# Agzs/BlockMaze

Hardware: AMD Instinct MI355X
Metric: Groth16 proofs/sec (send circuit, alt_bn128) (higher is better)
Workload: dtype u32 limbs (254-bit Fq/Fr Montgomery; all MSM accumulations, the H query's weighted bucket sum and the transforms' tiles on nine 29-bit limbs)

## Files before the change

### blockmaze_amd/csrc/msm.cuh

```cuda
#pragma once
#include <hip/hip_runtime.h>
#include "curve.cuh"

#include "field29.cuh"
namespace zk { struct MsmCounters { uint32_t n_ones; uint32_t n_other; uint32_t pad[2]; }; }
#include "htail29.cuh"
#include "oct29.cuh"
namespace zk {

constexpr int MSM_MAX_WINDOWS = 64;

__host__ __device__ inline int msm_num_windows(int c) { return 254 / c + 1; }

__device__ __forceinline__ void signed_digits(const uint32_t k[8], int c, int W, int *dig) {
  uint32_t carry = 0; const uint32_t half = 1u << (c - 1), full = 1u << c, mask = full - 1;
  for (int w = 0; w < W; w++) {
    int bit = w * c, word = bit >> 5, sh = bit & 31;
    uint64_t v = word < 8 ? k[word] : 0; if (word + 1 < 8) v |= (uint64_t)k[word + 1] << 32;
    uint32_t d = ((uint32_t)(v >> sh) & mask) + carry;
    if (d > half) { dig[w] = (int)d - (int)full; carry = 1; } else { dig[w] = (int)d; carry = 0; }
  }
}

template <int C, class Fn> __device__ __forceinline__ void for_each_digit(const uint32_t (&k)[8], Fn &&fn) {
// ... 12 lines not shown
}
constexpr uint32_t MSM_ENTRY_SIGN = 0x80000000u;


constexpr uint32_t MSM_LDS_HIST = 4096;
template <int C>
__global__ void __launch_bounds__(256) k_msm_classify(const Fr *__restrict__ scalars, const uint32_t *__restrict__ scalar_index,
    const uint8_t *__restrict__ point_is_inf,
                               uint32_t n, int c, int W, int filter_ones, uint32_t hist_stride, uint32_t n_hist, uint32_t *__restrict__ hist,
                                   uint32_t *__restrict__ ones, MsmCounters *cnt, MsmCounters *cnt_next) {
  __shared__ uint32_t lh[MSM_LDS_HIST]; const bool use_lds = n_hist <= MSM_LDS_HIST;
  if (blockIdx.x == 0 && threadIdx.x == 0) *cnt_next = MsmCounters{0, 0, {0, 0}};
  if (use_lds) { for (uint32_t b = threadIdx.x; b < n_hist; b += blockDim.x) lh[b] = 0; __syncthreads(); }
  uint32_t i = blockIdx.x * blockDim.x + threadIdx.x; bool live = i < n && !(point_is_inf && point_is_inf[i]); Fr k = Fr::zero();
  if (live) { k = scalars[scalar_index ? scalar_index[i] : i].from_mont(); live = !k.is_zero(); }
  bool is_one = false; if (live && filter_ones) { uint32_t o = k.l[0] ^ 1u; for (int j = 1; j < 8; j++) o |= k.l[j]; is_one = o == 0; }
  {
    uint64_t m = __ballot(is_one);
    if (m) {
      uint32_t lane = threadIdx.x & 63, base = 0;
      if (lane == (uint32_t)__ffsll((long long)m) - 1) base = atomicAdd(&cnt->n_ones, (uint32_t)__popcll(m));
      base = __shfl(base, __ffsll((long long)m) - 1, 64); if (is_one) ones[base + __popcll(m & ((1ull << lane) - 1))] = i; } }
  if (live && !is_one)
    msm_walk_digits<C>(k.l, c, W, [&](int w, int d) { if (d) { uint32_t key = (uint32_t)w * hist_stride + (uint32_t)(d < 0 ? -d : d) - 1;
        atomicAdd(use_lds ? &lh[key] : &hist[key], 1u); } });
  {
    uint64_t m = __ballot(live && !is_one);
    if (m && (threadIdx.x & 63) == (uint32_t)__ffsll((long long)m) - 1) atomicAdd(&cnt->n_other, (uint32_t)__popcll(m));
  }
  if (use_lds) { __syncthreads(); for (uint32_t b = threadIdx.x; b < n_hist; b += blockDim.x) if (lh[b]) atomicAdd(&hist[b], lh[b]); }
}

template <int C>
__global__ void __launch_bounds__(256) k_msm_scatter(const Fr *__restrict__ scalars, const uint32_t *__restrict__ scalar_index,
    const uint8_t *__restrict__ point_is_inf,
                              uint32_t n, int c, int W, int filter_ones, uint32_t hist_stride, uint32_t point_stride, uint32_t n_hist,
                                  const uint32_t *__restrict__ offsets, uint32_t *__restrict__ fill, uint32_t *__restrict__ entries) {
  __shared__ uint32_t lcnt[MSM_LDS_HIST], lbase[MSM_LDS_HIST]; const bool use_lds = n_hist <= MSM_LDS_HIST;
  if (use_lds) { for (uint32_t b = threadIdx.x; b < n_hist; b += blockDim.x) lcnt[b] = 0; __syncthreads(); }
  uint32_t i = blockIdx.x * blockDim.x + threadIdx.x; bool live = i < n && !(point_is_inf && point_is_inf[i]); Fr k = Fr::zero();
  if (live) { k = scalars[scalar_index ? scalar_index[i] : i].from_mont(); live = !k.is_zero(); }
  if (live && filter_ones) { uint32_t o = k.l[0] ^ 1u; for (int j = 1; j < 8; j++) o |= k.l[j]; if (o == 0) live = false; }
  auto entry_of = [&](int w, int d) {
    return (i + (uint32_t)w * point_stride) | (d < 0 ? MSM_ENTRY_SIGN : 0u);
  };
  if (!use_lds) {
    if (live) msm_walk_digits<C>(k.l, c, W, [&](int w, int d) { if (!d) return; uint32_t key = (uint32_t)w * hist_stride + (uint32_t)(d < 0 ? -d : d) - 1;
        entries[offsets[key] + atomicAdd(&fill[key], 1u)] = entry_of(w, d); });
    return;
  }
  if (live) msm_walk_digits<C>(k.l, c, W, [&](int w, int d) { if (d) atomicAdd(&lcnt[(uint32_t)w * hist_stride + (uint32_t)(d < 0 ? -d : d) - 1], 1u); });
  __syncthreads();
  for (uint32_t b = threadIdx.x; b < n_hist; b += blockDim.x) {
    const uint32_t m = lcnt[b];
    lbase[b] = m ? offsets[b] + atomicAdd(&fill[b], m) : 0;
    lcnt[b] = 0;
  }
  __syncthreads();
  if (live) msm_walk_digits<C>(k.l, c, W, [&](int w, int d) { if (!d) return; uint32_t key = (uint32_t)w * hist_stride + (uint32_t)(d < 0 ? -d : d) - 1;
      entries[lbase[key] + atomicAdd(&lcnt[key], 1u)] = entry_of(w, d); });
}

__host__ __device__ inline uint32_t hsort_spread(int c) { const int W = 254 / c + 1, tb = 254 - c * (W - 1); return tb < c - 2 && c * W > 256 ? 1u << (c * W - 256) : 1u; }
__host__ __device__ inline uint32_t hsort_multiple(uint32_t i, uint32_t spread) { return spread > 1 ? ((i * 2654435761u) >> 16) % spread : 0u; }
__device__ __forceinline__ void signed_digits9(const uint32_t k[9], int c, int W, int *dig) {
  uint32_t carry = 0; const uint32_t half = 1u << (c - 1), full = 1u << c, mask = full - 1;
  for (int w = 0; w < W; w++) {
    int bit = w * c, word = bit >> 5, sh = bit & 31;
    uint64_t v = word < 9 ? k[word] : 0; if (word + 1 < 9) v |= (uint64_t)k[word + 1] << 32;
    uint32_t d = ((uint32_t)(v >> sh) & mask) + carry;
    if (d > half) { dig[w] = (int)d - (int)full; carry = 1; } else { dig[w] = (int)d; carry = 0; }
  }
}
template <int C, class Fn> __device__ __forceinline__ void hsort_walk_digits(const uint32_t (&k)[8], uint32_t i, uint32_t spread, int c, int W, Fn &&fn) {
  if constexpr (C > 0) { msm_walk_digits<C>(k, c, W, fn); }
  else {
    const uint32_t m = hsort_multiple(i, spread); uint32_t k9[9]; uint64_t carry = 0;
#pragma unroll
    for (int j = 0; j < 8; j++) { const uint64_t t = (uint64_t)k[j] + (uint64_t)m * FrParams::MOD[j] + carry; k9[j] = (uint32_t)t; carry = t >> 32; }
    k9[8] = (uint32_t)carry;
    int dig[MSM_MAX_WINDOWS]; signed_digits9(k9, c, W, dig); for (int w = 0; w < W; w++) fn(w, dig[w]);
  }
}
constexpr uint32_t HSORT_GROUPS = 1024 , HSORT_BIN_THREADS = 256, HSORT_PER_THREAD = 2,
    HSORT_TILE = HSORT_BIN_THREADS * HSORT_PER_THREAD, HSORT_GROUP_THREADS = 1024, HSORT_MAX_PER_THREAD = 24, HSORT_SLICES = 8,
    HSORT_STAGE_W = 20 ;
struct HsortShape { uint32_t groups, low_bits, idx_bits, region; };
template <int C>
__global__ void __launch_bounds__(HSORT_BIN_THREADS) k_hsort_bin(const Fr *__restrict__ scalars, const Fr *__restrict__ mul_b, const Fr *__restrict__ mul_z,
    int z_is_table, const uint8_t *__restrict__ point_is_inf,
                                                                 uint32_t n, int c, int W, uint32_t point_stride, HsortShape sh, uint32_t spread,
                                                                     uint32_t *__restrict__ group_fill, uint32_t *__restrict__ mid, MsmCounters *cnt,
                                                                     MsmCounters *cnt_next) {
  zk_take_prio(sh.low_bits);
  __shared__ uint32_t lcnt[HSORT_GROUPS], lpos[HSORT_GROUPS], gbase[HSORT_GROUPS];
  __shared__ uint32_t stage[HSORT_TILE * HSORT_STAGE_W];
  __shared__ uint16_t stage_g[HSORT_TILE * HSORT_STAGE_W];
  __shared__ uint32_t wave_tot[HSORT_BIN_THREADS / 64];
  if (blockIdx.x == 0 && threadIdx.x == 0) *cnt_next = MsmCounters{0, 0, {0, 0}};
  for (uint32_t g = threadIdx.x; g < sh.groups; g += blockDim.x) lcnt[g] = 0;
  __syncthreads();
  Fr k[HSORT_PER_THREAD]; bool live[HSORT_PER_THREAD];
#pragma unroll
  for (int q = 0; q < (int)HSORT_PER_THREAD; q++) {
    const uint32_t i = blockIdx.x * HSORT_TILE + q * HSORT_BIN_THREADS + threadIdx.x;
    live[q] = i < n && !(point_is_inf && point_is_inf[i]);
    k[q] = Fr::zero();
    if (live[q]) { Fr v = scalars[i]; if (mul_b) v = v * mul_b[i] * mul_z[z_is_table ? i : 0]; k[q] = v.from_mont(); live[q] = !k[q].is_zero(); } }
  const uint32_t low_mask = (1u << sh.low_bits) - 1;
#pragma unroll
  for (int q = 0; q < (int)HSORT_PER_THREAD; q++) if (live[q]) hsort_walk_digits<C>(k[q].l, blockIdx.x * HSORT_TILE + q * HSORT_BIN_THREADS + threadIdx.x, spread, c, W, [&](int, int d) {
      if (d) atomicAdd(&lcnt[((uint32_t)(d < 0 ? -d : d) - 1) >> sh.low_bits], 1u); });
  __syncthreads();
  {
    uint32_t s = 0;
    const uint32_t per = (sh.groups + HSORT_BIN_THREADS - 1) / HSORT_BIN_THREADS, lo = threadIdx.x * per;
    for (uint32_t j = 0; j < per; j++) if (lo + j < sh.groups) s += lcnt[lo + j];
    uint32_t inc = s; for (int d = 1; d < 64; d <<= 1) { uint32_t t = __shfl_up(inc, d, 64); if ((int)(threadIdx.x & 63) >= d) inc += t; }
    if ((threadIdx.x & 63) == 63) wave_tot[threadIdx.x >> 6] = inc;
    __syncthreads();
    uint32_t ex = inc - s; for (uint32_t wv = 0; wv < (threadIdx.x >> 6); wv++) ex += wave_tot[wv];
    bool over = false;
    for (uint32_t j = 0; j < per; j++) if (lo + j < sh.groups) {
      const uint32_t g = lo + j, m = lcnt[g];
      lpos[g] = ex;
      ex += m;
      const uint32_t b = m ? atomicAdd(&group_fill[g], m) : 0;
      if (b + m > sh.region) over = true;
      gbase[g] = b;
    }
    if (over) atomicOr(&cnt->pad[0], 1u); }
  __syncthreads();
  for (uint32_t g = threadIdx.x; g < sh.groups; g += blockDim.x) lcnt[g] = lpos[g];
  __syncthreads();
#pragma unroll
  for (int q = 0; q < (int)HSORT_PER_THREAD; q++) if (live[q]) { const uint32_t i = blockIdx.x * HSORT_TILE + q * HSORT_BIN_THREADS + threadIdx.x;
    hsort_walk_digits<C>(k[q].l, i, spread, c, W, [&](int w, int d) { if (!d) return; const uint32_t key = (uint32_t)(d < 0 ? -d : d) - 1, g = key >> sh.low_bits,
        p = atomicAdd(&lcnt[g], 1u);
      if (p < HSORT_TILE * HSORT_STAGE_W) { stage[p] = ((key & low_mask) << (sh.idx_bits + 1)) | ((d < 0 ? 1u : 0u) << sh.idx_bits) | (i +
          (uint32_t)w * point_stride); stage_g[p] = (uint16_t)g; } }); }
  __syncthreads();
  const uint32_t total = min(lcnt[sh.groups - 1], HSORT_TILE * HSORT_STAGE_W);
  for (uint32_t p = threadIdx.x; p < total; p += blockDim.x) {
    const uint32_t g = stage_g[p], pos = gbase[g] + (p - lpos[g]);
    if (pos < sh.region) mid[(size_t)g * sh.region + pos] = stage[p];
  }
}
static __global__ void __launch_bounds__(HSORT_GROUP_THREADS) k_hsort_group(const uint32_t *__restrict__ mid, uint32_t *__restrict__ group_fill, HsortShape sh,
    uint32_t *__restrict__ entries, uint32_t *__restrict__ counts, uint32_t *__restrict__ offsets,
                                                                            uint32_t *__restrict__ group_n) {
  zk_take_prio(sh.low_bits);
  __shared__ uint32_t lcnt[1024], lpre[1024];
  const uint32_t g = blockIdx.x, nb = 1u << sh.low_bits, n_g = min(group_fill[g], sh.region); const uint32_t *src = mid + (size_t)g * sh.region;
  for (uint32_t b = threadIdx.x; b < nb; b += blockDim.x) lcnt[b] = 0;
  __syncthreads();
  if (threadIdx.x == 0) {
    group_fill[g] = 0;
    group_n[g] = n_g;
  }
  uint32_t e[HSORT_MAX_PER_THREAD]; int ne = 0;
#pragma unroll
  for (int j = 0; j < (int)HSORT_MAX_PER_THREAD; j++) {
    const uint32_t p = (uint32_t)j * HSORT_GROUP_THREADS + threadIdx.x;
    if (p < n_g) {
      e[j] = src[p];
      atomicAdd(&lcnt[e[j] >> (sh.idx_bits + 1)], 1u);
      ne = j + 1;
    }
  }
  __syncthreads();
  if (threadIdx.x < 64) {
    const uint32_t per = (nb + 63) / 64, lo = threadIdx.x * per; uint32_t s = 0; for (uint32_t j = 0; j < per; j++) if (lo + j < nb) s += lcnt[lo + j];
    uint32_t inc = s; for (int d = 1; d < 64; d <<= 1) { uint32_t t = __shfl_up(inc, d, 64); if ((int)threadIdx.x >= d) inc += t; }
    uint32_t ex = inc - s; for (uint32_t j = 0; j < per; j++) if (lo + j < nb) { lpre[lo + j] = ex; ex += lcnt[lo + j]; } }
  __syncthreads();
  for (uint32_t b = threadIdx.x; b < nb; b += blockDim.x) {
    const uint32_t bucket = (g << sh.low_bits) | b;
    counts[bucket] = lcnt[b];
    offsets[bucket] = g * sh.region + lpre[b];
    lcnt[b] = 0;
  }
  __syncthreads();
  uint32_t *dst = entries + (size_t)g * sh.region;
  extern __shared__ uint32_t hsg_stage[];
#pragma unroll
  for (int j = 0; j < (int)HSORT_MAX_PER_THREAD; j++) if (j < ne) {
    const uint32_t v = e[j], b = v >> (sh.idx_bits + 1), r = atomicAdd(&lcnt[b], 1u);
    hsg_stage[lpre[b] + r] = v;
  }
  __syncthreads();
  for (uint32_t p = threadIdx.x; p < n_g; p += blockDim.x) dst[p] = hsg_stage[p];
}

static __global__ void k_fr_mul3(const Fr *__restrict__ a, const Fr *__restrict__ b, const Fr *__restrict__ z, int z_is_table, uint32_t n,
    Fr *__restrict__ out) {
  uint32_t i = blockIdx.x * blockDim.x + threadIdx.x; if (i < n) out[i] = a[i] * b[i] * z[z_is_table ? i : 0];
}

constexpr int SCAN_BLOCK = 1024, SCAN_ITEMS = 4;
static __global__ void k_scan_local(const uint32_t *__restrict__ in, uint32_t *__restrict__ out, uint32_t *__restrict__ block_sums, uint32_t n) {
  __shared__ uint32_t sh[SCAN_BLOCK]; uint32_t base = blockIdx.x * SCAN_BLOCK * SCAN_ITEMS + threadIdx.x * SCAN_ITEMS; uint32_t v[SCAN_ITEMS], s = 0;
  for (int j = 0; j < SCAN_ITEMS; j++) { v[j] = base + j < n ? in[base + j] : 0; s += v[j]; }
  sh[threadIdx.x] = s; __syncthreads();
  for (int d = 1; d < SCAN_BLOCK; d <<= 1) { uint32_t t = threadIdx.x >= d ? sh[threadIdx.x - d] : 0; __syncthreads(); sh[threadIdx.x] += t; __syncthreads(); }
  uint32_t excl = sh[threadIdx.x] - s;
  for (int j = 0; j < SCAN_ITEMS; j++) { if (base + j < n) out[base + j] = excl; excl += v[j]; }
  if (threadIdx.x == SCAN_BLOCK - 1) block_sums[blockIdx.x] = sh[SCAN_BLOCK - 1];
}
static __global__ void k_scan_block_sums(uint32_t *block_sums, uint32_t nblocks) {
  __shared__ uint32_t sh[SCAN_BLOCK]; uint32_t carry = 0;
  for (uint32_t base = 0; base < nblocks; base += SCAN_BLOCK) {
    uint32_t i = base + threadIdx.x, v = i < nblocks ? block_sums[i] : 0; sh[threadIdx.x] = v; __syncthreads();
    for (int d = 1; d < SCAN_BLOCK; d <<= 1) {
      uint32_t t = threadIdx.x >= d ? sh[threadIdx.x - d] : 0;
      __syncthreads();
      sh[threadIdx.x] += t;
      __syncthreads();
    }
    if (i < nblocks) block_sums[i] = carry + sh[threadIdx.x] - v; uint32_t tot = sh[SCAN_BLOCK - 1]; __syncthreads(); carry += tot;
  }
}
static __global__ void k_scan_add(uint32_t *__restrict__ out, const uint32_t *__restrict__ block_sums, uint32_t n) {
  uint32_t base = blockIdx.x * SCAN_BLOCK * SCAN_ITEMS + threadIdx.x * SCAN_ITEMS, add = block_sums[blockIdx.x];
  for (int j = 0; j < SCAN_ITEMS; j++) if (base + j < n) out[base + j] += add;
}

template <class P> __device__ __forceinline__ Fp<P> shfl_down_struct(const Fp<P> &v, int delta) {
  Fp<P> r;
#pragma unroll
  for (int i = 0; i < 8; i++) r.l[i] = __shfl_down(v.l[i], delta, 64);
  return r;
}
__device__ __forceinline__ Fq2 shfl_down_struct(const Fq2 &v, int delta) { return {shfl_down_struct(v.c0, delta), shfl_down_struct(v.c1, delta)}; }
template <class F> __device__ __forceinline__ XYZZ<F> shfl_down_struct(const XYZZ<F> &v, int delta) {
  return {shfl_down_struct(v.X, delta), shfl_down_struct(v.Y, delta), shfl_down_struct(v.ZZ, delta), shfl_down_struct(v.ZZZ, delta)};
}

constexpr uint32_t MSM_TASK = 16;
constexpr uint32_t BSORT_CLASSES = 64, BSORT_BLOCK = 256;
__device__ __forceinline__ uint32_t bsort_class(uint32_t count) { return BSORT_CLASSES - 1 - min(count, BSORT_CLASSES - 1); }
static __global__ void __launch_bounds__(BSORT_BLOCK) k_bsort_hist(uint32_t *__restrict__ counts, uint32_t n_buckets, uint32_t n_blocks,
    uint32_t *__restrict__ block_hist, uint32_t clip) {
  __shared__ uint32_t h[BSORT_CLASSES]; if (threadIdx.x < BSORT_CLASSES) h[threadIdx.x] = 0; __syncthreads();
  uint32_t b = blockIdx.x * BSORT_BLOCK + threadIdx.x;
  if (b < n_buckets) {
    uint32_t cv = counts[b];
    if (clip && cv > clip) {
      cv = clip;
      counts[b] = cv;
    }
    atomicAdd(&h[bsort_class(cv)], 1u);
  }
  __syncthreads();
  if (threadIdx.x < BSORT_CLASSES) block_hist[threadIdx.x * n_blocks + blockIdx.x] = h[threadIdx.x];
}
static __global__ void __launch_bounds__(BSORT_BLOCK) k_bsort_scatter(const uint32_t *__restrict__ counts, uint32_t n_buckets, uint32_t n_blocks,
    const uint32_t *__restrict__ block_off,
                                                               uint32_t *__restrict__ order, uint32_t *__restrict__ rank_of, uint32_t *__restrict__ ntasks,
                                                                   uint32_t *__restrict__ cls_start, uint4 *__restrict__ bucket_mem, uint32_t bucket_u4) {
  __shared__ uint32_t h[BSORT_CLASSES]; if (threadIdx.x < BSORT_CLASSES) h[threadIdx.x] = 0; __syncthreads();
  uint32_t b = blockIdx.x * BSORT_BLOCK + threadIdx.x;
  if (b < n_buckets) {
    uint32_t cnt = counts[b], cls = bsort_class(cnt), pos = block_off[cls * n_blocks + blockIdx.x] + atomicAdd(&h[cls], 1u);
    order[pos] = b;
    rank_of[b] = pos;
    ntasks[pos] = (cnt + MSM_TASK - 1) / MSM_TASK;
    if (cnt == 0) for (uint32_t j = 0; j < bucket_u4; j++) bucket_mem[(size_t)b * bucket_u4 + j] = make_uint4(0, 0, 0, 0);
  }
  if (b == 0) ntasks[n_buckets] = 0;
  if (blockIdx.x == 0 && threadIdx.x < BSORT_CLASSES) cls_start[threadIdx.x] = block_off[threadIdx.x * n_blocks];
}
// ... 707 lines not shown
```

### blockmaze_amd/csrc/msm_impl.hpp

```cpp
#pragma once
#include <cstring>
#include <memory>
#include <atomic>
#include <cstdio>
#include "gpu_internal.hpp"

#define ZK_MSM_DISPATCH_C(cval, CALL) do { if ((cval) == 8) { ZK_MSM_CHECK_C(8); CALL(8); } else if ((cval) == 16) { ZK_MSM_CHECK_C(16); CALL(16); } else { CALL(0); } } while (0)
#define ZK_MSM_CHECK_C(CC) do { if (c != (CC) || W != msm_num_windows(CC)) throw GpuError("msm: compiled-in digit walk launched with a different window size"); } while (0)

namespace zk {
struct WsortBuffers { uint32_t NB = 0, cap = 0; size_t n = 0; DevBuf<uint32_t> fill , entries , ones ,
    counters ; int parity = 0; bool shared = false; hipEvent_t sorted = nullptr; int leader_stream = -1;
  ~WsortBuffers() { if (sorted) hipEventDestroy(sorted); } };
template <class F, class RawAffine>
struct MsmImpl {
  size_t n; int c, W, WB; uint32_t NB;
  bool filter_ones; uint32_t seg, n_ones_quads; std::string label = "msm"; int stream_id = -1;
  struct Bases { size_t n = 0; int c = 0, W = 0, WB = 0; bool any_inf = false, table261_only = false ; DevBuf<RawAffine> points,
      points261 , groups261 , ones_groups ;
      DevBuf<uint8_t> inf;
    };
  std::shared_ptr<const Bases> bases; const DevBuf<RawAffine> &points; const DevBuf<uint8_t> &inf; bool any_inf = false;
  bool split_ones = false;
  hipStream_t ones_stream = nullptr;
// ... 258 lines not shown
    if (!hsort) throw GpuError("msm: run_product needs the one-pass sort");
    prod_b = b;
    prod_z = z;
    prod_z_table = z_is_table;
    run_impl(a, nullptr);
  }
  void run(const Fe32 *scalars, const uint32_t *scalar_index) { prod_b = nullptr; tagged = false; run_impl(scalars, scalar_index); }
  void run_tagged(const Fe32 *z_all_, const WitnessTags &wt, const uint32_t *scalar_index) {
    prod_b = nullptr; wtags = wt; z_all = z_all_; tagged = wt.tags != nullptr && wt.other_vars != nullptr;
    run_impl(scalar_index ? z_all_ : z_all_ + wt.base, scalar_index); }

  void run_impl(const Fe32 *scalars, const uint32_t *scalar_index) {
    hipStream_t s = stream();
    size_t nbk = (size_t)WB * NB;
    const uint32_t hist_stride = WB == 1 ? 0 : NB, point_stride = WB == 1 && W > 1 ? (uint32_t)n : 0;
    const uint8_t *infp = any_inf ? inf.get() : nullptr;
    const uint32_t bucket_u4 = sizeof(XYZZ<F>) / 16; XYZZ<F> *res = (XYZZ<F> *)res_dev;
    parity ^= 1; MsmCounters *cnt = counters();
    bool ones_forked = false;
    auto ones_path = [&](hipStream_t os) { Stage st((label + ".ones").c_str(), os); uint32_t g = cdiv(n_ones_quads, GROUP);
      hipLaunchKernelGGL((k_msm_sum_ones<F>), dim3(cdiv((size_t)n_ones_quads * 4, 256)), dim3(256), 0, os, (const Affine<F> *)points.get(), ones.get(), cnt,
          n_ones_quads, (XYZZ<F> *)ones_partial.get());
      hipLaunchKernelGGL((k_xyzz_group_sum<F>), dim3(g), dim3(256), 0, os, (const XYZZ<F> *)ones_partial.get(), GROUP, n_ones_quads, (XYZZ<F> *)ones_l2.get(),
          (uint4 *)nullptr, (uint4 *)nullptr);
      hipLaunchKernelGGL((k_xyzz_group_sum<F>), dim3(1), dim3(256), 0, os, (const XYZZ<F> *)ones_l2.get(), g, g, res + RS, (uint4 *)nullptr, (uint4 *)nullptr);
    };
    last_scalars = scalars; last_index = scalar_index;
    if (wfused) {
      parity ^= 1;
      WsortBuffers &w = *ws; MsmCounters *wc = (MsmCounters *)w.counters.get();
      if (ws_leader) {
        w.parity ^= 1;
        w.leader_stream = stream_id;
        Stage st((label + ".sort").c_str(), s);
        const uint8_t *winf = w.shared ? nullptr : infp;
        if (tagged) {
          const uint32_t ones_blocks = cdiv(n, 256), other_blocks = cdiv(wtags.n_other, 256);
#define ZK_CALL(CC) hipLaunchKernelGGL(k_wsort_tagged<CC>, dim3(ones_blocks + other_blocks), dim3(256), 0, s, (const Fr *)z_all, wtags, scalar_index, winf, (uint32_t)n, c, W, point_stride, NB, w.cap, ones_blocks, w.fill.get() + (size_t)w.parity * NB, w.fill.get() + (size_t)(w.parity ^ 1) * NB, w.entries.get(), w.ones.get(), wc + w.parity, wc + (w.parity ^ 1))
          ZK_MSM_DISPATCH_C(c, ZK_CALL);
#undef ZK_CALL
        } else {
#define ZK_CALL(CC) hipLaunchKernelGGL(k_wsort<CC>, dim3(cdiv(n, 256)), dim3(256), 0, s, (const Fr *)scalars, scalar_index, winf, (uint32_t)n, c, W, point_stride, NB, w.cap, w.fill.get() + (size_t)w.parity * NB, w.fill.get() + (size_t)(w.parity ^ 1) * NB, w.entries.get(), w.ones.get(), wc + w.parity, wc + (w.parity ^ 1))
        ZK_MSM_DISPATCH_C(c, ZK_CALL);
#undef ZK_CALL
        }
        if (w.shared) HIP_CHECK(hipEventRecord(w.sorted, s)); }
      else if (w.leader_stream != stream_id) HIP_CHECK(hipStreamWaitEvent(s, w.sorted, 0));
      uint4 *cdst = (uint4 *)(res + RS + 1);
      const uint32_t *fl = w.fill.get() + (size_t)w.parity * NB;
      const uint32_t top = 31 - (uint32_t)__builtin_clz(NB);
      const dim3 lanes_grid((WFUSED_BUCKET_LANES + WFUSED_ONES_LANES) / 256), fold_grid(NB + WFUSED_ONES_GROUPS);
      if constexpr (sizeof(F) == 32) {
        Point29Rec *p1 = (Point29Rec *)partials.get(), *p2 = (Point29Rec *)ones_partial.get();
        { Stage st((label + ".accumulate").c_str(), s);
          hipLaunchKernelGGL(k_wacc_lanes29<0>, lanes_grid, dim3(256), 0, s, (const Affine<Fq> *)bases->points261.get(),
              (const Affine<Fq> *)bases->groups261.get(), w.entries.get(), fl, w.cap, zk_with_prio(NB, ZKP_WLANES), w.ones.get(), wc + w.parity, p1, lane_off.get());
          hipLaunchKernelGGL(k_wfold29<0>, fold_grid, dim3(256), 0, s, (const Point29Rec *)p1, (const uint32_t *)lane_off.get(), zk_with_prio(NB, ZKP_WIT),
              (uint32_t)WFUSED_BUCKET_LANES, p2);
        }
        { Stage st((label + ".reduce").c_str(), s);
          hipLaunchKernelGGL(k_wtail29<0>, dim3(top + 2), dim3(256), 0, s, (const Point29Rec *)p2, zk_with_prio(NB, ZKP_WIT), (const Point29Rec *)p2 + NB,
              (uint32_t)WFUSED_ONES_GROUPS, (uint32_t)WTAIL_SLOTS, (XYZZ<Fq> *)res, wc + w.parity, cdst, ws_leader ? 0u : 16u);
        }
      } else {
        Point29Rec2 *p1 = (Point29Rec2 *)partials.get(), *p2 = (Point29Rec2 *)ones_partial.get();
        { Stage st((label + ".accumulate").c_str(), s);
          hipLaunchKernelGGL(k_wacc_lanes_g2_29<0>, lanes_grid, dim3(256), 0, s, (const Affine<Fq2> *)bases->points261.get(),
              (const Affine<Fq2> *)bases->groups261.get(), w.entries.get(), fl, w.cap, zk_with_prio(NB, ZKP_WLANES), w.ones.get(), wc + w.parity, p1, lane_off.get());
          hipLaunchKernelGGL(k_wfold_g2_29<0>, fold_grid, dim3(OCT_BLOCK), 0, s, (const Point29Rec2 *)p1, (const uint32_t *)lane_off.get(), zk_with_prio(NB, ZKP_WIT),
              (uint32_t)WFUSED_BUCKET_LANES, p2);
        }
        { Stage st((label + ".reduce").c_str(), s);
          hipLaunchKernelGGL(k_wtail_g2_29<0>, dim3(top + 2), dim3(OCT_BLOCK), 0, s, (const Point29Rec2 *)p2, zk_with_prio(NB, ZKP_WIT), (const Point29Rec2 *)p2 + NB,
              (uint32_t)WFUSED_ONES_GROUPS, (uint32_t)WTAIL_SLOTS, (XYZZ<Fq2> *)res, wc + w.parity, cdst, ws_leader ? 0u : 16u);
        }
      }
      return;
    }
    const bool hs_run = hsort && scalar_index == nullptr;
    if (hs_run) {
      if constexpr (sizeof(F) == 32) {
      { Stage st((label + ".sort").c_str(), s);
        HsortShape hs_prio = hs; hs_prio.low_bits |= zk_prio_bits(ZKP_HSORT);
#define ZK_CALL(CC) hipLaunchKernelGGL(k_hsort_bin<CC>, dim3(cdiv(n, HSORT_TILE)), dim3(HSORT_BIN_THREADS), 0, s, (const Fr *)scalars, (const Fr *)prod_b, (const Fr *)prod_z, (int)prod_z_table, infp, (uint32_t)n, c, W, point_stride, hs_prio, (CC) ? 1u : hsort_spread(c), group_fill.get(), mid.get(), cnt, counters_next())
        ZK_MSM_DISPATCH_C(c, ZK_CALL);
#undef ZK_CALL
        static std::atomic<uint64_t> lds_done{0}; zk_raise_dynamic_lds(reinterpret_cast<const void *>(&k_hsort_group), 128 * 1024, lds_done);
        hipLaunchKernelGGL(k_hsort_group, dim3(hs.groups), dim3(HSORT_GROUP_THREADS), 4 * hs.region, s, (const uint32_t *)mid.get(), group_fill.get(), hs_prio, entries.get(),
            hist(), offsets.get(), group_n.get());
      }
      {
        Stage st((label + ".accumulate").c_str(), s);
        const uint32_t h_run = crowded ? std::max(this->h_run, h_run_crowded) : this->h_run;
        const dim3 grid(cdiv(cdiv(n * (size_t)W, h_run) + hs.groups, 256));
        if (any_inf) hipLaunchKernelGGL(k_hacc_runs29<1>, grid, dim3(256), 0, s, (const Affine<Fq> *)bases->points261.get(), entries.get(), group_n.get(),
            offsets.get(), hs, h_run, zk_with_prio(h_maxp, ZKP_HACC), (Piece29 *)partials.get(), cnt);
        else hipLaunchKernelGGL(k_hacc_runs29<0>, grid, dim3(256), 0, s, (const Affine<Fq> *)bases->points261.get(), entries.get(), group_n.get(),
            offsets.get(), hs, h_run, zk_with_prio(h_maxp, ZKP_HACC), (Piece29 *)partials.get(), cnt);
      }
      {
        Stage st((label + ".combine").c_str(), s);
        const uint32_t h_run = crowded ? std::max(this->h_run, h_run_crowded) : this->h_run;
        const size_t pieces = n * (size_t)W / NB / h_run;
        const uint32_t ll = pieces > 40 ? 3 : pieces > 18 ? 2 : 1;
        last_ll = ll;
        hipLaunchKernelGGL(k_hacc_combine29, dim3(cdiv(nbk << ll, 256)), dim3(256), 0, s, (const Piece29 *)partials.get(), offsets.get(), hist(), hs, h_run,
            h_maxp, (uint32_t)nbk, zk_with_prio(ll, ZKP_HTAIL), (XYZZ<Fq> *)bucket_array(), htail29 ? (Point29Rec *)hb29.get() : nullptr, cnt);
      }
      }
    } else
    { Stage st((label + ".sort").c_str(), s);
      if (hsort) throw GpuError("msm: the group-binned sort takes no scalar index");
#define ZK_CALL(CC) hipLaunchKernelGGL(k_msm_classify<CC>, dim3(cdiv(n, 256)), dim3(256), 0, s, (const Fr *)scalars, scalar_index, infp, (uint32_t)n, c, W, (int)filter_ones, hist_stride, (uint32_t)nbk, hist(), ones.get(), cnt, counters_next())
      if (n) ZK_MSM_DISPATCH_C(c, ZK_CALL);
#undef ZK_CALL
      if (filter_ones && n && split_ones) {
        HIP_CHECK(hipEventRecord(ev_classified, s));
        HIP_CHECK(hipStreamWaitEvent(ones_stream, ev_classified, 0));
        ones_path(ones_stream);
        HIP_CHECK(hipEventRecord(ev_ones, ones_stream));
        ones_forked = true;
      }
      if (nbk <= PLAN_SMALL_MAX) {
        hipLaunchKernelGGL(k_msm_plan_small, dim3(1), dim3(PLAN_THREADS), 0, s, hist(), (uint32_t)nbk, offsets.get(), order.get(), rank_of.get(),
            task_off.get(), cls_start.get(), (uint4 *)bucket_array(), bucket_u4);
      } else {
        scanner.run(hist(), offsets.get(), nbk, s);
        hipLaunchKernelGGL(k_bsort_hist, dim3(bsort_blocks), dim3(BSORT_BLOCK), 0, s, hist(), (uint32_t)nbk, bsort_blocks, block_hist.get(), 0u);
        bsort_scanner->run(block_hist.get(), block_off.get(), (size_t)bsort_blocks * BSORT_CLASSES, s);
        hipLaunchKernelGGL(k_bsort_scatter, dim3(bsort_blocks), dim3(BSORT_BLOCK), 0, s, hist(), (uint32_t)nbk, bsort_blocks, block_off.get(), order.get(),
            rank_of.get(), ntasks.get(), cls_start.get(), (uint4 *)bucket_array(), bucket_u4);
        task_scanner.run(ntasks.get(), task_off.get(), nbk + 1, s);
      }
#define ZK_CALL(CC) hipLaunchKernelGGL(k_msm_scatter<CC>, dim3(cdiv(n, 256)), dim3(256), 0, s, (const Fr *)scalars, scalar_index, infp, (uint32_t)n, c, W, (int)filter_ones, hist_stride, point_stride, (uint32_t)nbk, offsets.get(), fill(), entries.get())
      if (n) ZK_MSM_DISPATCH_C(c, ZK_CALL);
#undef ZK_CALL
    }
    if (!hs_run) {
      { Stage st((label + ".accumulate").c_str(), s);
        if (bases->table261_only) hipLaunchKernelGGL((k_msm_accumulate_tasks<F, 1>), dim3(cdiv(max_tasks, 256)), dim3(256), 0, s, (const Affine<F> *)bases->points261.get(), entries.get(),
            offsets.get(), hist(), order.get(), task_off.get(), (uint32_t)nbk, max_tasks, MSM_TASK, bucket_array(), (XYZZ<F> *)partials.get());
        else hipLaunchKernelGGL((k_msm_accumulate_tasks<F, 0>), dim3(cdiv(max_tasks, 256)), dim3(256), 0, s, (const Affine<F> *)points.get(), entries.get(),
            offsets.get(), hist(), order.get(), task_off.get(), (uint32_t)nbk, max_tasks, MSM_TASK, bucket_array(), (XYZZ<F> *)partials.get());
      }
      { Stage st((label + ".combine").c_str(), s);
        hipLaunchKernelGGL((k_msm_combine_tasks<F>), dim3(HEAVY_BLOCKS + cdiv(nbk, 64)), dim3(256), 0, s, order.get(), task_off.get(), cls_start.get(),
            HEAVY_BLOCKS, (const XYZZ<F> *)partials.get(), bucket_array(), zeroed.get(), (uint32_t)(2 * nbk), 0);
      }
    }
    if (bitsum && hs_run && htail29) {
      if constexpr (sizeof(F) == 32) {
        Stage st_red((label + ".reduce").c_str(), s);
      const HtailShape ts = htail_shape(NB);
      const uint32_t marg_block = std::max(1u << ts.hi_bits, (1u << ts.lo_bits) / ts.row_chunks) <= 128 ? 64 : 256;
      hipLaunchKernelGGL(k_hmarg29<0>, dim3(htail_marg_blocks(ts)), dim3(marg_block), 0, s, (const Point29Rec *)hb29.get(), zk_with_prio(NB, ZKP_HTAIL), (Point29Rec *)hmarg.get());
      hipLaunchKernelGGL(k_hbits29<0>, dim3(ts.top + 1), dim3(256), 0, s, (const Point29Rec *)hmarg.get(), zk_with_prio(NB, ZKP_HTAIL), (XYZZ<Fq> *)res, cnt, (uint4 *)(res + RS + 1));
    }
  }
    else { Stage st_red((label + ".reduce").c_str(), s);
      if (RS > WB) memset(h_result + (size_t)WB * sizeof(XYZZ<F>), 0, (size_t)(RS - WB) * sizeof(XYZZ<F>));
      uint32_t spw = NB / seg, nseg = (uint32_t)WB * spw; uint4 *csrc = (uint4 *)cnt; uint4 *cdst = (uint4 *)(res + RS + 1);
      hipLaunchKernelGGL((k_msm_reduce_segments<F>), dim3(cdiv(nseg, 16)), dim3(64), 0, s, (const XYZZ<F> *)bucket_array(), NB, seg, nseg,
          (XYZZ<F> *)seg_out.get());
      if (spw > GROUP) { uint32_t g = spw / GROUP;
        hipLaunchKernelGGL((k_xyzz_group_sum<F>), dim3(WB * g), dim3(256), 0, s, (const XYZZ<F> *)seg_out.get(), GROUP, nseg, (XYZZ<F> *)seg_l2.get(),
            (uint4 *)nullptr, (uint4 *)nullptr);
        hipLaunchKernelGGL((k_xyzz_group_sum<F>), dim3(WB), dim3(256), 0, s, (const XYZZ<F> *)seg_l2.get(), g, (uint32_t)WB * g, res, csrc, cdst);
// ... 21 lines not shown
```

Measured before the change: 1341.

## Restructure hsort binning with biased branchless digits and dynamic LDS staging

The bin kernel now runs one scalar per thread with 512 threads. It adds a precomputed bias so signed-window digits come out branchless from the biased scalar, and caches each digit once in registers instead of walking the digits twice. LDS staging moves to dynamic shared memory sized by the actual window count, and the scatter uses a single per-group delta instead of two lookups. The group kernel switches to a full-block prefix scan and splits the atomic slot claim from the staging writes. The risks are higher register pressure from the per-digit arrays, lower occupancy with the larger dynamic LDS, and possible mismatch with the old carry-based digit semantics.

```diff
diff --git a/blockmaze_amd/csrc/msm.cuh b/blockmaze_amd/csrc/msm.cuh
--- a/blockmaze_amd/csrc/msm.cuh
+++ b/blockmaze_amd/csrc/msm.cuh
@@ -118,68 +118,112 @@
     int dig[MSM_MAX_WINDOWS]; signed_digits9(k9, c, W, dig); for (int w = 0; w < W; w++) fn(w, dig[w]);
   }
 }
-constexpr uint32_t HSORT_GROUPS = 1024 , HSORT_BIN_THREADS = 256, HSORT_PER_THREAD = 2,
+constexpr uint32_t HSORT_GROUPS = 1024 , HSORT_BIN_THREADS = 512, HSORT_PER_THREAD = 1,
     HSORT_TILE = HSORT_BIN_THREADS * HSORT_PER_THREAD, HSORT_GROUP_THREADS = 1024, HSORT_MAX_PER_THREAD = 24, HSORT_SLICES = 8,
     HSORT_STAGE_W = 20 ;
 struct HsortShape { uint32_t groups, low_bits, idx_bits, region; };
+struct HsortBias { uint32_t w[9]; };
+__host__ __device__ constexpr HsortBias hsort_bias(int c) {
+  HsortBias b{}; const int W = 254 / c + 1;
+  for (int w = 0; w < W; w++) {
+    const int bit = c * w, word = bit >> 5; const uint64_t v = (uint64_t)((1u << (c - 1)) - 1) << (bit & 31);
+    if (word < 9) b.w[word] |= (uint32_t)v;
+    if (word + 1 < 9) b.w[word + 1] |= (uint32_t)(v >> 32);
+  }
+  return b;
+}
+constexpr uint32_t HSORT_NO_DIGIT = 0xffffffffu;
+__host__ __device__ inline uint32_t hsort_bin_lds_bytes(uint32_t groups, int W) { return 8 * groups + 6 * HSORT_TILE * (uint32_t)W; }
 template <int C>
 __global__ void __launch_bounds__(HSORT_BIN_THREADS) k_hsort_bin(const Fr *__restrict__ scalars, const Fr *__restrict__ mul_b, const Fr *__restrict__ mul_z,
     int z_is_table, const uint8_t *__restrict__ point_is_inf,
                                                                  uint32_t n, int c, int W, uint32_t point_stride, HsortShape sh, uint32_t spread,
-                                                                     uint32_t *__restrict__ group_fill, uint32_t *__restrict__ mid, MsmCounters *cnt,
-                                                                     MsmCounters *cnt_next) {
+                                                                     HsortBias bias, uint32_t *__restrict__ group_fill, uint32_t *__restrict__ mid,
+                                                                     MsmCounters *cnt, MsmCounters *cnt_next) {
   zk_take_prio(sh.low_bits);
-  __shared__ uint32_t lcnt[HSORT_GROUPS], lpos[HSORT_GROUPS], gbase[HSORT_GROUPS];
-  __shared__ uint32_t stage[HSORT_TILE * HSORT_STAGE_W];
-  __shared__ uint16_t stage_g[HSORT_TILE * HSORT_STAGE_W];
-  __shared__ uint32_t wave_tot[HSORT_BIN_THREADS / 64];
+  constexpr int WMAX = C ? 254 / (C ? C : 1) + 1 : (int)HSORT_STAGE_W;
+  extern __shared__ uint32_t hsb_lds[];
+  const uint32_t cap = HSORT_TILE * (uint32_t)W;
+  uint32_t *const lcnt = hsb_lds, *const delta = lcnt + sh.groups, *const stage = delta + sh.groups; uint16_t *const stage_g = (uint16_t *)(stage + cap);
+  __shared__ uint32_t wave_tot[HSORT_BIN_THREADS / 64], tile_total;
   if (blockIdx.x == 0 && threadIdx.x == 0) *cnt_next = MsmCounters{0, 0, {0, 0}};
   for (uint32_t g = threadIdx.x; g < sh.groups; g += blockDim.x) lcnt[g] = 0;
   __syncthreads();
-  Fr k[HSORT_PER_THREAD]; bool live[HSORT_PER_THREAD];
-#pragma unroll
-  for (int q = 0; q < (int)HSORT_PER_THREAD; q++) {
-    const uint32_t i = blockIdx.x * HSORT_TILE + q * HSORT_BIN_THREADS + threadIdx.x;
-    live[q] = i < n && !(point_is_inf && point_is_inf[i]);
-    k[q] = Fr::zero();
-    if (live[q]) { Fr v = scalars[i]; if (mul_b) v = v * mul_b[i] * mul_z[z_is_table ? i : 0]; k[q] = v.from_mont(); live[q] = !k[q].is_zero(); } }
-  const uint32_t low_mask = (1u << sh.low_bits) - 1;
-#pragma unroll
-  for (int q = 0; q < (int)HSORT_PER_THREAD; q++) if (live[q]) hsort_walk_digits<C>(k[q].l, blockIdx.x * HSORT_TILE + q * HSORT_BIN_THREADS + threadIdx.x, spread, c, W, [&](int, int d) {
-      if (d) atomicAdd(&lcnt[((uint32_t)(d < 0 ? -d : d) - 1) >> sh.low_bits], 1u); });
-  __syncthreads();
+  const uint32_t i = blockIdx.x * HSORT_TILE + threadIdx.x;
+  bool live = i < n && !(point_is_inf && point_is_inf[i]);
+  uint32_t kb[9] = {0, 0, 0, 0, 0, 0, 0, 0, 0};
+  if (live) {
+    Fr v = scalars[i]; if (mul_b) v = v * mul_b[i] * mul_z[z_is_table ? i : 0];
+    const Fr k = v.from_mont(); live = !k.is_zero();
+    const uint32_t m = C > 0 ? 0u : hsort_multiple(i, spread); uint64_t carry = 0;
+#pragma unroll
+    for (int j = 0; j < 8; j++) {
+      uint64_t t = (uint64_t)k.l[j] + carry;
+      if constexpr (C > 0) t += hsort_bias(C ? C : 1).w[j]; else t += (uint64_t)m * FrParams::MOD[j] + bias.w[j];
+      kb[j] = (uint32_t)t; carry = t >> 32;
+    }
+    kb[8] = (uint32_t)carry + (C > 0 ? hsort_bias(C ? C : 1).w[8] : bias.w[8]);
+  }
+  const uint32_t low_mask = (1u << sh.low_bits) - 1, cc = C > 0 ? (uint32_t)C : (uint32_t)c, dmask = (1u << cc) - 1, dbias = (1u << (cc - 1)) - 1;
+  uint32_t dk[WMAX];
+#pragma unroll
+  for (int w = 0; w < WMAX; w++) {
+    uint32_t raw;
+    if constexpr (C > 0) {
+      const int bit = w * C, word = bit >> 5, s = bit & 31;
+      raw = word < 9 ? kb[word < 9 ? word : 0] >> s : 0u; if (s + C > 32 && word + 1 < 9) raw |= kb[word + 1 < 9 ? word + 1 : 0] << (32 - s);
+    } else {
+      raw = kb[0];
+#pragma unroll
+      for (int j = 0; j < 8; j++) kb[j] = (kb[j] >> cc) | (kb[j + 1] << (32 - cc));
+      kb[8] >>= cc;
+    }
+    const int d = (int)(raw & dmask) - (int)dbias;
+    dk[w] = live && d != 0 && (C > 0 || w < W) ? ((uint32_t)(d < 0 ? -d : d) - 1) | (d < 0 ? 0x80000000u : 0u) : HSORT_NO_DIGIT;
+    if (dk[w] != HSORT_NO_DIGIT) atomicAdd(&lcnt[(dk[w] & 0x7fffffffu) >> sh.low_bits], 1u);
+  }
+  __syncthreads();
+  const uint32_t per = (sh.groups + HSORT_BIN_THREADS - 1) / HSORT_BIN_THREADS, lo = threadIdx.x * per;
+  uint32_t gm[HSORT_GROUPS / HSORT_BIN_THREADS], gb[HSORT_GROUPS / HSORT_BIN_THREADS];
   {
     uint32_t s = 0;
-    const uint32_t per = (sh.groups + HSORT_BIN_THREADS - 1) / HSORT_BIN_THREADS, lo = threadIdx.x * per;
     for (uint32_t j = 0; j < per; j++) if (lo + j < sh.groups) s += lcnt[lo + j];
     uint32_t inc = s; for (int d = 1; d < 64; d <<= 1) { uint32_t t = __shfl_up(inc, d, 64); if ((int)(threadIdx.x & 63) >= d) inc += t; }
     if ((threadIdx.x & 63) == 63) wave_tot[threadIdx.x >> 6] = inc;
     __syncthreads();
     uint32_t ex = inc - s; for (uint32_t wv = 0; wv < (threadIdx.x >> 6); wv++) ex += wave_tot[wv];
+#pragma unroll
+    for (uint32_t j = 0; j < HSORT_GROUPS / HSORT_BIN_THREADS; j++) { gm[j] = 0; gb[j] = 0; if (j < per && lo + j < sh.groups) {
+      const uint32_t g = lo + j, m = lcnt[g];
+      lcnt[g] = ex; delta[g] = 0u - ex;
+      ex += m; gm[j] = m;
+      if (m) gb[j] = atomicAdd(&group_fill[g], m);
+    } }
+    if (threadIdx.x == HSORT_BIN_THREADS - 1) tile_total = ex; }
+  __syncthreads();
+  {
+    uint32_t p[WMAX];
+#pragma unroll
+    for (int w = 0; w < WMAX; w++) p[w] = dk[w] != HSORT_NO_DIGIT ? atomicAdd(&lcnt[(dk[w] & 0x7fffffffu) >> sh.low_bits], 1u) : cap;
+#pragma unroll
+    for (int w = 0; w < WMAX; w++) if (p[w] < cap) {
+      const uint32_t key = dk[w] & 0x7fffffffu;
+      stage[p[w]] = ((key & low_mask) << (sh.idx_bits + 1)) | ((dk[w] >> 31) << sh.idx_bits) | (i + (uint32_t)w * point_stride);
+      stage_g[p[w]] = (uint16_t)(key >> sh.low_bits);
+    }
+  }
+  {
     bool over = false;
-    for (uint32_t j = 0; j < per; j++) if (lo + j < sh.groups) {
-      const uint32_t g = lo + j, m = lcnt[g];
-      lpos[g] = ex;
-      ex += m;
-      const uint32_t b = m ? atomicAdd(&group_fill[g], m) : 0;
-      if (b + m > sh.region) over = true;
-      gbase[g] = b;
-    }
-    if (over) atomicOr(&cnt->pad[0], 1u); }
-  __syncthreads();
-  for (uint32_t g = threadIdx.x; g < sh.groups; g += blockDim.x) lcnt[g] = lpos[g];
-  __syncthreads();
-#pragma unroll
-  for (int q = 0; q < (int)HSORT_PER_THREAD; q++) if (live[q]) { const uint32_t i = blockIdx.x * HSORT_TILE + q * HSORT_BIN_THREADS + threadIdx.x;
-    hsort_walk_digits<C>(k[q].l, i, spread, c, W, [&](int w, int d) { if (!d) return; const uint32_t key = (uint32_t)(d < 0 ? -d : d) - 1, g = key >> sh.low_bits,
-        p = atomicAdd(&lcnt[g], 1u);
-      if (p < HSORT_TILE * HSORT_STAGE_W) { stage[p] = ((key & low_mask) << (sh.idx_bits + 1)) | ((d < 0 ? 1u : 0u) << sh.idx_bits) | (i +
-          (uint32_t)w * point_stride); stage_g[p] = (uint16_t)g; } }); }
-  __syncthreads();
-  const uint32_t total = min(lcnt[sh.groups - 1], HSORT_TILE * HSORT_STAGE_W);
-  for (uint32_t p = threadIdx.x; p < total; p += blockDim.x) {
-    const uint32_t g = stage_g[p], pos = gbase[g] + (p - lpos[g]);
-    if (pos < sh.region) mid[(size_t)g * sh.region + pos] = stage[p];
+#pragma unroll
+    for (uint32_t j = 0; j < HSORT_GROUPS / HSORT_BIN_THREADS; j++) if (gm[j]) { delta[lo + j] += gb[j]; if (gb[j] + gm[j] > sh.region) over = true; }
+    if (over) atomicOr(&cnt->pad[0], 1u);
+  }
+  __syncthreads();
+  const uint32_t total = min(tile_total, cap);
+#pragma unroll 4
+  for (uint32_t q = threadIdx.x; q < total; q += HSORT_BIN_THREADS) {
+    const uint32_t g = stage_g[q], v = stage[q], pos = delta[g] + q;
+    if (pos < sh.region) mid[(size_t)g * sh.region + pos] = v;
   }
 }
 static __global__ void __launch_bounds__(HSORT_GROUP_THREADS) k_hsort_group(const uint32_t *__restrict__ mid, uint32_t *__restrict__ group_fill, HsortShape sh,
@@ -194,35 +238,36 @@
     group_fill[g] = 0;
     group_n[g] = n_g;
   }
+  __shared__ uint32_t wave_tot[HSORT_GROUP_THREADS / 64];
   uint32_t e[HSORT_MAX_PER_THREAD]; int ne = 0;
 #pragma unroll
   for (int j = 0; j < (int)HSORT_MAX_PER_THREAD; j++) {
     const uint32_t p = (uint32_t)j * HSORT_GROUP_THREADS + threadIdx.x;
-    if (p < n_g) {
-      e[j] = src[p];
-      atomicAdd(&lcnt[e[j] >> (sh.idx_bits + 1)], 1u);
-      ne = j + 1;
-    }
-  }
-  __syncthreads();
-  if (threadIdx.x < 64) {
-    const uint32_t per = (nb + 63) / 64, lo = threadIdx.x * per; uint32_t s = 0; for (uint32_t j = 0; j < per; j++) if (lo + j < nb) s += lcnt[lo + j];
-    uint32_t inc = s; for (int d = 1; d < 64; d <<= 1) { uint32_t t = __shfl_up(inc, d, 64); if ((int)threadIdx.x >= d) inc += t; }
-    uint32_t ex = inc - s; for (uint32_t j = 0; j < per; j++) if (lo + j < nb) { lpre[lo + j] = ex; ex += lcnt[lo + j]; } }
-  __syncthreads();
-  for (uint32_t b = threadIdx.x; b < nb; b += blockDim.x) {
-    const uint32_t bucket = (g << sh.low_bits) | b;
-    counts[bucket] = lcnt[b];
-    offsets[bucket] = g * sh.region + lpre[b];
-    lcnt[b] = 0;
+    if (p < n_g) { e[j] = src[p]; ne = j + 1; }
+  }
+#pragma unroll
+  for (int j = 0; j < (int)HSORT_MAX_PER_THREAD; j++) if (j < ne) atomicAdd(&lcnt[e[j] >> (sh.idx_bits + 1)], 1u);
+  __syncthreads();
+  const uint32_t my = threadIdx.x < nb ? lcnt[threadIdx.x] : 0;
+  uint32_t inc = my; for (int d = 1; d < 64; d <<= 1) { uint32_t t = __shfl_up(inc, d, 64); if ((int)(threadIdx.x & 63) >= d) inc += t; }
+  if ((threadIdx.x & 63) == 63) wave_tot[threadIdx.x >> 6] = inc;
+  __syncthreads();
+  if (threadIdx.x < nb) {
+    uint32_t ex = inc - my; for (uint32_t wv = 0; wv < (threadIdx.x >> 6); wv++) ex += wave_tot[wv];
+    const uint32_t bucket = (g << sh.low_bits) | threadIdx.x;
+    counts[bucket] = my;
+    offsets[bucket] = g * sh.region + ex;
+    lpre[threadIdx.x] = ex;
   }
   __syncthreads();
   uint32_t *dst = entries + (size_t)g * sh.region;
   extern __shared__ uint32_t hsg_stage[];
-#pragma unroll
-  for (int j = 0; j < (int)HSORT_MAX_PER_THREAD; j++) if (j < ne) {
-    const uint32_t v = e[j], b = v >> (sh.idx_bits + 1), r = atomicAdd(&lcnt[b], 1u);
-    hsg_stage[lpre[b] + r] = v;
+  {
+    uint32_t at[HSORT_MAX_PER_THREAD];
+#pragma unroll
+    for (int j = 0; j < (int)HSORT_MAX_PER_THREAD; j++) if (j < ne) at[j] = atomicAdd(&lpre[e[j] >> (sh.idx_bits + 1)], 1u);
+#pragma unroll
+    for (int j = 0; j < (int)HSORT_MAX_PER_THREAD; j++) if (j < ne) hsg_stage[at[j]] = e[j];
   }
   __syncthreads();
   for (uint32_t p = threadIdx.x; p < n_g; p += blockDim.x) dst[p] = hsg_stage[p];
diff --git a/blockmaze_amd/csrc/msm_impl.hpp b/blockmaze_amd/csrc/msm_impl.hpp
--- a/blockmaze_amd/csrc/msm_impl.hpp
+++ b/blockmaze_amd/csrc/msm_impl.hpp
@@ -364,7 +364,7 @@
       if constexpr (sizeof(F) == 32) {
       { Stage st((label + ".sort").c_str(), s);
         HsortShape hs_prio = hs; hs_prio.low_bits |= zk_prio_bits(ZKP_HSORT);
-#define ZK_CALL(CC) hipLaunchKernelGGL(k_hsort_bin<CC>, dim3(cdiv(n, HSORT_TILE)), dim3(HSORT_BIN_THREADS), 0, s, (const Fr *)scalars, (const Fr *)prod_b, (const Fr *)prod_z, (int)prod_z_table, infp, (uint32_t)n, c, W, point_stride, hs_prio, (CC) ? 1u : hsort_spread(c), group_fill.get(), mid.get(), cnt, counters_next())
+#define ZK_CALL(CC) static std::atomic<uint64_t> bin_lds_done{0}; zk_raise_dynamic_lds(reinterpret_cast<const void *>(&k_hsort_bin<CC>), 96 * 1024, bin_lds_done); hipLaunchKernelGGL(k_hsort_bin<CC>, dim3(cdiv(n, HSORT_TILE)), dim3(HSORT_BIN_THREADS), hsort_bin_lds_bytes(hs.groups, W), s, (const Fr *)scalars, (const Fr *)prod_b, (const Fr *)prod_z, (int)prod_z_table, infp, (uint32_t)n, c, W, point_stride, hs_prio, (CC) ? 1u : hsort_spread(c), hsort_bias(c), group_fill.get(), mid.get(), cnt, counters_next())
         ZK_MSM_DISPATCH_C(c, ZK_CALL);
 #undef ZK_CALL
         static std::atomic<uint64_t> lds_done{0}; zk_raise_dynamic_lds(reinterpret_cast<const void *>(&k_hsort_group), 128 * 1024, lds_done);
```

Measured after the change: 1259. 6.2% lower.
